# someone-in-somewhere/multimodal_rag

Hardware: AMD Instinct MI355X
Metric: chunks embedded/sec + queries/sec top_k=5 over 1M×768 at 1/2/4/8 GPUs (higher is better)
Workload: dtype f16

## Files before the change

multimodal_rag_amd/csrc/search_qsw.hip:

```cpp
#include "search_shared.h"

#include <type_traits>
#include <utility>

using namespace mmrag;

namespace mmrag_impl {

namespace {

template <typename F, int... I>
__device__ __forceinline__ void static_for_impl(F &&f, std::integer_sequence<int, I...>) {
    (f(std::integral_constant<int, I>{}), ...);
}
template <int N, typename F>
__device__ __forceinline__ void static_for(F &&f) {
    static_for_impl(f, std::make_integer_sequence<int, N>{});
}

constexpr int QSW_XCH = 2048 + 64;
constexpr int qsw_lists_bytes(int K, int MS) { return K * (MS == 32 ? 2 : 4) * QS_QROWS * 8; }

constexpr SlabRing qsw_ring(int NK, int K, int MS) {
#if defined(MMRAG_QSW_RING16)
    if (MS == 16 && NK % (MMRAG_QSW_RING16 / 10) == 0) return SlabRing{MMRAG_QSW_RING16 / 10, MMRAG_QSW_RING16 % 10};
#endif
    return slab_ring(NK, qsw_lists_bytes(K, MS) + QSW_XCH);
}

#define MMRAG_QSW_S32(MNEMONIC, QC, C00, C01, C10, C11, ACC)                                                  \
    asm volatile("v_xad_u32 %[t], %[lo], %[xc], %[st]\n\t"                                                    \
                 "ds_read_b128 %[n0], %[t] offset:%[o0]\n\t"                                                  \
                 "ds_read_b128 %[n1], %[t] offset:%[o1]\n\t" MNEMONIC " %[c00], %[a0], %[q0], " C00 "\n\t"    \
                 MNEMONIC " %[c01], %[a0], %[q1], " C01 "\n\t" MNEMONIC " %[c10], %[a1], %[q0], " C10 "\n\t"  \
                 MNEMONIC " %[c11], %[a1], %[q1], " C11 "\n\t"                                                \
                 "s_waitcnt lgkmcnt(0)"                                                                       \
                 : [c00] ACC(c00), [c01] ACC(c01), [c10] ACC(c10), [c11] ACC(c11), [n0] "=&v"(n0),            \
                   [n1] "=&v"(n1), [t] "=&v"(tmp)                                                             \
                 : [a0] "v"(a0), [a1] "v"(a1), [q0] QC(q0), [q1] QC(q1), [lo] "v"(lo), [st] "s"(st),          \
                   [xc] "i"(XC), [o0] "i"(OFF0), [o1] "i"(OFF1))

template <int DT, bool QA, bool FIRST, int XC, int OFF0, int OFF1, typename FT>
__device__ __forceinline__ void qsw_stmt32(f32x16_t &c00, f32x16_t &c01, f32x16_t &c10, f32x16_t &c11, const FT a0,
                                           const FT a1, const FT q0, const FT q1, FT &n0, FT &n1, const unsigned lo,
                                           const unsigned st) {
    unsigned tmp;
    if constexpr (FIRST) {
        static_assert(QA, "the first k-step's Q fragments live in the accumulator file");
        if constexpr (DT == MMRAG_F16) MMRAG_QSW_S32("v_mfma_f32_32x32x16_f16", "a", "0", "0", "0", "0", "=&v");
        else MMRAG_QSW_S32("v_mfma_f32_32x32x16_bf16", "a", "0", "0", "0", "0", "=&v");
    } else if constexpr (DT == MMRAG_F16) {
        if constexpr (QA) MMRAG_QSW_S32("v_mfma_f32_32x32x16_f16", "a", "%[c00]", "%[c01]", "%[c10]", "%[c11]", "+v");
        else MMRAG_QSW_S32("v_mfma_f32_32x32x16_f16", "v", "%[c00]", "%[c01]", "%[c10]", "%[c11]", "+v");
    } else {
        if constexpr (QA) MMRAG_QSW_S32("v_mfma_f32_32x32x16_bf16", "a", "%[c00]", "%[c01]", "%[c10]", "%[c11]", "+v");
        else MMRAG_QSW_S32("v_mfma_f32_32x32x16_bf16", "v", "%[c00]", "%[c01]", "%[c10]", "%[c11]", "+v");
    }
}

#define MMRAG_QSW_S16(MNEMONIC, QC, D0, D1, D2, D3, D4, D5, D6, D7, ACC)                                      \
    asm volatile(MNEMONIC " %[d0], %[a0], %[q0], " D0 "\n\t"                                                  \
                 "ds_read_b128 %[n0], %[ad] offset:%[o0]\n\t" MNEMONIC " %[d1], %[a0], %[q1], " D1 "\n\t"     \
                 "ds_read_b128 %[n1], %[ad] offset:%[o1]\n\t" MNEMONIC " %[d2], %[a0], %[q2], " D2 "\n\t"     \
                 MNEMONIC " %[d3], %[a0], %[q3], " D3 "\n\t" MNEMONIC " %[d4], %[a1], %[q0], " D4 "\n\t"      \
                 MNEMONIC " %[d5], %[a1], %[q1], " D5 "\n\t" MNEMONIC " %[d6], %[a1], %[q2], " D6 "\n\t"      \
                 MNEMONIC " %[d7], %[a1], %[q3], " D7 "\n\t"                                                  \
                 "s_waitcnt lgkmcnt(0)"                                                                       \
                 : [d0] ACC(d0), [d1] ACC(d1), [d2] ACC(d2), [d3] ACC(d3), [d4] ACC(d4), [d5] ACC(d5),        \
                   [d6] ACC(d6), [d7] ACC(d7), [n0] "=&v"(n0), [n1] "=&v"(n1)                                 \
                 : [a0] "v"(a0), [a1] "v"(a1), [q0] QC(q0), [q1] QC(q1), [q2] QC(q2), [q3] QC(q3),            \
                   [ad] "v"(adr), [o0] "i"(OFF0), [o1] "i"(OFF1))
#define MMRAG_QSW_S16_ACC(MNEMONIC, QC)                                                                       \
    MMRAG_QSW_S16(MNEMONIC, QC, "%[d0]", "%[d1]", "%[d2]", "%[d3]", "%[d4]", "%[d5]", "%[d6]", "%[d7]", "+v")
#define MMRAG_QSW_S16_FIRST(MNEMONIC, QC) MMRAG_QSW_S16(MNEMONIC, QC, "0", "0", "0", "0", "0", "0", "0", "0", "=&v")

template <int DT, bool QA, bool FIRST, int OFF0, int OFF1, typename FT>
__device__ __forceinline__ void qsw_stmt16(f32x4_t &d0, f32x4_t &d1, f32x4_t &d2, f32x4_t &d3, f32x4_t &d4,
                                           f32x4_t &d5, f32x4_t &d6, f32x4_t &d7, const FT a0, const FT a1,
                                           const FT q0, const FT q1, const FT q2, const FT q3, FT &n0, FT &n1,
                                           const unsigned adr) {
    if constexpr (FIRST) {
        static_assert(QA, "the first k-step's Q fragments live in the accumulator file");
        if constexpr (DT == MMRAG_F16) MMRAG_QSW_S16_FIRST("v_mfma_f32_16x16x32_f16", "a");
        else MMRAG_QSW_S16_FIRST("v_mfma_f32_16x16x32_bf16", "a");
    } else if constexpr (DT == MMRAG_F16) {
        if constexpr (QA) MMRAG_QSW_S16_ACC("v_mfma_f32_16x16x32_f16", "a");
        else MMRAG_QSW_S16_ACC("v_mfma_f32_16x16x32_f16", "v");
    } else {
        if constexpr (QA) MMRAG_QSW_S16_ACC("v_mfma_f32_16x16x32_bf16", "a");
        else MMRAG_QSW_S16_ACC("v_mfma_f32_16x16x32_bf16", "v");
    }
}

__device__ __forceinline__ void qsw_stage_addr(unsigned &a_lo, unsigned &a_hi, const unsigned lo, const unsigned st) {
    asm volatile("v_add_u32 %0, %2, %3\n\tv_xad_u32 %1, %2, 64, %3" : "=&v"(a_lo), "=&v"(a_hi) : "v"(lo), "s"(st));
}

__device__ __forceinline__ float max16_raw(float x0, float x1, float x2, float x3, float x4, float x5, float x6, float x7,
                                           float x8, float x9, float x10, float x11, float x12, float x13, float x14,
                                           float x15) {
    float r;
    asm("v_max3_f32 %0, %1, %2, %3\n\t"
        "v_max3_f32 %0, %0, %4, %5\n\t"
        "v_max3_f32 %0, %0, %6, %7\n\t"
        "v_max3_f32 %0, %0, %8, %9\n\t"
        "v_max3_f32 %0, %0, %10, %11\n\t"
        "v_max3_f32 %0, %0, %12, %13\n\t"
        "v_max3_f32 %0, %0, %14, %15\n\t"
        "v_max_f32 %0, %0, %16"
        : "=&v"(r)
        : "v"(x0), "v"(x1), "v"(x2), "v"(x3), "v"(x4), "v"(x5), "v"(x6), "v"(x7), "v"(x8), "v"(x9), "v"(x10), "v"(x11),
          "v"(x12), "v"(x13), "v"(x14), "v"(x15));
    return r;
}

constexpr int CP_SC1 = 16;

}

template <int DT, int NK, int K, int MS, bool NT>
__global__ __launch_bounds__(256, 1) void cosine_topk_walk_kernel(const KParams p) {
#if defined(__HIP_DEVICE_COMPILE__)
    using FT = typename FragType<DT>::T;
    static_assert(MS == 32 || MS == 16, "MFMA shape");
    constexpr int R = QS_TILE_ROWS;
    static_assert(R == 64, "statements are written for 64-row tiles");
    constexpr int RB = R / 32;
    constexpr int SLABB = R * SLAB;
    constexpr int NQB = MS == 32 ? 2 : 4;
    constexpr int QW = MS;
    constexpr int NSUB = 64 / QW;
    constexpr int NGRP = 16 / NSUB;
    constexpr SlabRing RING = qsw_ring(NK, K, MS);
    constexpr int G = RING.G, NST = RING.NST;
    constexpr int SPT = NK / G;
    constexpr int STAGE = G * SLABB;
    constexpr int PPS = G * RB;
    constexpr int KSTG = G * 4;
    constexpr int KST = MS == 32 ? NK * 4 : NK * 2;
    constexpr int QA_STEPS = 64 / NQB;
    constexpr int LISTS = qsw_lists_bytes(K, MS);
    constexpr int LOOK = (NST + 1 + SPT - 1) / SPT + 1;
    static_assert(NST >= 3 && NST * STAGE + LISTS + QSW_XCH <= 160 * 1024, "LDS");
    static_assert((NST - 1) * PPS <= 56, "vmcnt range");
    static_assert((G - 1) * SLABB + 48 * SLAB + 2048 < 65536, "ds_read immediate offset");
    static_assert(2 * PPS == KSTG, "one piece after every other statement");
    constexpr int LANDT = ((NST - 2) * PPS + 1 + SPT * PPS - 1) / (SPT * PPS);
    static_assert(LANDT >= 1 && LANDT * SPT * PPS - 1 >= (NST - 2) * PPS, "exchange pieces land before they are used");
    static_assert(LOOK <= 6, "ticket slots");

    __shared__ __attribute__((aligned(1024))) char smem[NST * STAGE + LISTS + QSW_XCH];
    float *lists = (float *)(smem + NST * STAGE);
    float *const gather_lds = (float *)(smem + NST * STAGE + LISTS);
    float *const poll_lds = (float *)(smem + NST * STAGE + LISTS + 1024);
    int *const tk_lds = (int *)(smem + NST * STAGE + LISTS + 2048);

    const int tid = threadIdx.x;
    const int lane = tid & 63;
    const int wave = __builtin_amdgcn_readfirstlane(tid >> 6);
    const int ql = lane & (QW - 1);
    const int sub = lane / QW;
    auto dev_dbg = [&](unsigned flag) -> bool {
#if defined(MMRAG_QSW_DEV)
        return (p.dbg & flag) != 0;
#else
        (void)flag;
        return false;
#endif
    };
    const unsigned long long t_entry = (p.dbg & DBG_QS_CLOCK) ? __builtin_amdgcn_s_memrealtime() : 0ull;

    const unsigned RBy = p.row_bytes;
    const int walkers = p.walkers;
    const int bx = (int)blockIdx.x % walkers;
    const int by = (int)blockIdx.x / walkers;
    const int q0 = by * QS_QROWS;
    const int p_static = p.p_static;
    auto pos_tile = [&](int pos) -> int {
        if (pos < p_static) return bx + pos * walkers;
        return p_static * walkers + (int)((unsigned)__builtin_amdgcn_readfirstlane(tk_lds[pos & 7]) - TICKET0);
    };

    unsigned c_off0;
    {
        const int row = (wave * RB) * 8 + (lane >> 3);
        c_off0 = (unsigned)row * RBy + (unsigned)(((lane & 7) ^ ((row >> 1) & 7)) * 16);
    }
    auto c_off = [&](int i) -> unsigned { return i == 0 ? c_off0 : (c_off0 ^ 64u) + 8u * RBy; };
    int is_pos = 0;
    int fill_tile = bx;
    __amdgpu_buffer_rsrc_t fill_rsrc;
    typedef __attribute__((address_space(3))) char *lds_char_t;
    const lds_char_t wave_lds = (lds_char_t)(lds_ptr_t)(smem + wave * (RB * 1024));
    lds_char_t stage_lds = wave_lds;
    auto fill_open = [&]() {
        const bool real = (unsigned)fill_tile < (unsigned)p.n_tiles && !dev_dbg(DBG_QS_NO_DMA);
        const long long row0 = real ? (dev_dbg(DBG_QS_DMA_L2) ? (long long)bx * R : (long long)fill_tile * R) : 0;
        const long long rows_left = p.n - row0;
        const unsigned c_bytes = real ? (unsigned)((rows_left < R ? rows_left : (long long)R) * (long long)RBy) : 0u;
        fill_rsrc = __builtin_amdgcn_make_buffer_rsrc((void *)(p.corpus + (size_t)row0 * RBy), 0, c_bytes, 0x00020000);
    };
    auto next_fill = [&](auto is_sg_c, int buf) {
        constexpr int IS_SG = decltype(is_sg_c)::value;
        if constexpr (IS_SG == 0) {
            if (is_pos != 0) fill_tile = pos_tile(is_pos);
            fill_open();
            ++is_pos;
        }
        stage_lds = wave_lds + buf * STAGE;
        asm volatile("" : "+s"(stage_lds));
    };
    unsigned koff = 0;
    auto issue_piece = [&](auto is_sg_c, auto pi_c) {
        constexpr int IS_SG = decltype(is_sg_c)::value, PI = decltype(pi_c)::value;
        constexpr int g = PI / RB, i = PI % RB;
        if constexpr (i == 0) asm volatile("s_movk_i32 %0, %1" : "=s"(koff) : "n"((IS_SG * G + g) * SLAB));
        __builtin_amdgcn_raw_ptr_buffer_load_lds(fill_rsrc, (lds_ptr_t)(stage_lds + g * SLABB + i * 1024), 16, c_off(i),
                                                 koff, 0, NT ? 2 : 0);
    };

    const bool any_tile = bx < p.n_tiles;
    if (any_tile)
        static_for<NST>([&](auto st_c) {
            constexpr int st = decltype(st_c)::value;
            next_fill(std::integral_constant<int, st % SPT>{}, st);
            static_for<PPS>([&](auto pi_c) { issue_piece(std::integral_constant<int, st % SPT>{}, pi_c); });
        });
    asm volatile("s_movk_i32 %0, %1" : "=s"(koff) : "n"(((NST - 1) % SPT) * G * SLAB));

    FT qf[NQB][KST];
    float thr[NQB];
    static_for<NQB>([&](auto qb_c) {
        constexpr int qb = decltype(qb_c)::value;
        const int qrow = q0 + wave * 64 + qb * QW + ql;
        const bool live = qrow < p.B;
        const char *src = p.q + (size_t)(live ? qrow : 0) * RBy + sub * 16;
#pragma unroll
        for (int s = 0; s < KST; ++s) {
            FT v = *(const FT *)(src + s * (16 * NSUB));
            if (!live) v = FT{};
            qf[qb][s] = v;
        }
        thr[qb] = !live ? INFINITY : NEG_INF;
    });
    float *const my_lists = lists + tid;
    auto lst_v = [&](int qb, int i) -> float & { return my_lists[(qb * 2 * K + i) * QS_QROWS]; };
    auto lst_r = [&](int qb, int i) -> int & { return *(int *)&my_lists[(qb * 2 * K + K + i) * QS_QROWS]; };
#pragma unroll
    for (int qb = 0; qb < NQB; ++qb)
#pragma unroll
        for (int i = 0; i < K; ++i) {
            lst_v(qb, i) = NEG_INF;
            lst_r(qb, i) = INT_MAX;
        }

    const int sw = (ql >> 1) & 7;
    const unsigned lane_off0 = (unsigned)(ql * SLAB + ((sub ^ sw) * 16));
    const unsigned lane_off64 = lane_off0 ^ 64u;
    const unsigned smem_base = (unsigned)(size_t)(lds_ptr_t)smem;

    auto lane_now = []() -> int {
        int l;
        asm volatile("v_mbcnt_lo_u32_b32 %0, -1, 0\n\tv_mbcnt_hi_u32_b32 %0, -1, %0" : "=v"(l));
        return l;
    };
    f32x16_t c32[MS == 32 ? 4 : 1];
    f32x4_t c16[MS == 16 ? 16 : 1];
    auto score = [&](auto qb_c, auto gi_c, int i) -> float {
        constexpr int qb = decltype(qb_c)::value, gi = decltype(gi_c)::value;
        if constexpr (MS == 32) return c32[(gi >> 2) * 2 + qb][4 * (gi & 3) + i];
        else return c16[gi * 4 + qb][i];
    };
    auto grp_row = [](int gi) -> int { return MS == 32 ? (gi >> 2) * 32 + 8 * (gi & 3) : gi * 16; };
    auto strike = [&](unsigned m0, unsigned m1, const int sub) {
        static_for<NQB>([&](auto qb_c) {
            static_for<NGRP>([&](auto gi_c) {
                constexpr int qb = decltype(qb_c)::value, gi = decltype(gi_c)::value;
                constexpr int r0 = MS == 32 ? (gi >> 2) * 32 + 8 * (gi & 3) : gi * 16;
                const unsigned m = (r0 < 32 ? m0 : m1) >> ((r0 & 31) + 4 * sub);
#pragma unroll
                for (int i = 0; i < 4; ++i) {
                    const bool ok = (m >> i) & 1u;
                    if constexpr (MS == 32) {
                        constexpr int a = (gi >> 2) * 2 + qb, e = 4 * (gi & 3);
                        c32[a][e + i] = ok ? c32[a][e + i] : NEG_INF;
                    } else {
                        c16[gi * 4 + qb][i] = ok ? c16[gi * 4 + qb][i] : NEG_INF;
                    }
                }
            });
        });
    };

    auto select = [&](auto qb_c, const int row_base, float *const my_lists) {
        auto lst_v = [&](int qb, int i) -> float & { return my_lists[(qb * 2 * K + i) * QS_QROWS]; };
        auto lst_r = [&](int qb, int i) -> int & { return *(int *)&my_lists[(qb * 2 * K + K + i) * QS_QROWS]; };
        constexpr int qb = decltype(qb_c)::value;
        auto max16 = [&](auto g0_c) -> float {
            constexpr int g0 = decltype(g0_c)::value;
            using G0 = std::integral_constant<int, g0>;
            using G1 = std::integral_constant<int, g0 + 1>;
            using G2 = std::integral_constant<int, g0 + 2>;
            using G3 = std::integral_constant<int, g0 + 3>;
            return max16_raw(score(qb_c, G0{}, 0), score(qb_c, G0{}, 1), score(qb_c, G0{}, 2), score(qb_c, G0{}, 3),
                             score(qb_c, G1{}, 0), score(qb_c, G1{}, 1), score(qb_c, G1{}, 2), score(qb_c, G1{}, 3),
                             score(qb_c, G2{}, 0), score(qb_c, G2{}, 1), score(qb_c, G2{}, 2), score(qb_c, G2{}, 3),
                             score(qb_c, G3{}, 0), score(qb_c, G3{}, 1), score(qb_c, G3{}, 2), score(qb_c, G3{}, 3));
        };
        float mx = max16(std::integral_constant<int, 0>{});
        if constexpr (NGRP == 8) mx = fmaxf(mx, max16(std::integral_constant<int, 4>{}));
        float t = thr[qb];
        if (__builtin_amdgcn_ballot_w64(mx >= t) == 0ull) return;
        constexpr int NE = NGRP * 4;
        float bar = t;
        if (__builtin_amdgcn_ballot_w64(t == NEG_INF) != 0ull) {
            float prev = INFINITY;
#pragma unroll
            for (int r = 0; r < K; ++r) {
                float m = NEG_INF;
                static_for<NGRP>([&](auto gi_c) {
                    const float x0 = score(qb_c, gi_c, 0), x1 = score(qb_c, gi_c, 1);
                    const float x2 = score(qb_c, gi_c, 2), x3 = score(qb_c, gi_c, 3);
                    const float y0 = x0 < prev ? x0 : NEG_INF, y1 = x1 < prev ? x1 : NEG_INF;
                    const float y2 = x2 < prev ? x2 : NEG_INF, y3 = x3 < prev ? x3 : NEG_INF;
                    m = fmaxf(m, fmaxf(fmaxf(y0, y1), fmaxf(y2, y3)));
                });
                prev = m;
            }
            bar = fmaxf(t, prev);
        }
        unsigned mask = 0;
        static_for<NE>([&](auto e_c) {
            constexpr int e = decltype(e_c)::value;
            mask |= score(qb_c, std::integral_constant<int, e / 4>{}, e % 4) >= bar ? (1u << e) : 0u;
        });
        TopList<K> L;
#pragma unroll
        for (int i = 0; i < K; ++i) {
            L.v[i] = lst_v(qb, i);
            L.r[i] = lst_r(qb, i);
        }
        constexpr int DENSE_AT = NE == 16 ? 8 : 12;
        if (__builtin_amdgcn_ballot_w64(__builtin_popcount(mask) > DENSE_AT) == 0ull) {
            while (__builtin_amdgcn_ballot_w64(mask != 0u) != 0ull) {
                const bool valid = mask != 0u;
                const unsigned e = (unsigned)__builtin_ctz(mask | (1u << (NE - 1)));
                mask &= mask - 1u;
                float lvl[NE];
                static_for<NE>([&](auto e_c) {
                    constexpr int x = decltype(e_c)::value;
                    lvl[x] = score(qb_c, std::integral_constant<int, x / 4>{}, x % 4);
                });
#pragma unroll
                for (int w = NE / 2, b = 0; w >= 1; w >>= 1, ++b) {
                    const bool bit = (e >> b) & 1u;
#pragma unroll
                    for (int i = 0; i < w; ++i) lvl[i] = bit ? lvl[2 * i + 1] : lvl[2 * i];
                }
                const float sc = lvl[0];
                const int row = MS == 32 ? (int)(((e >> 4) << 5) + (((e >> 2) & 3u) << 3) + (e & 3u))
                                         : (int)(((e >> 2) << 4) + (e & 3u));
                L.insert_strict_flat(valid && sc >= t ? sc : NEG_INF, row_base + row);
                t = fmaxf(t, L.v[K - 1]);
            }
        } else {
            static_for<NGRP>([&](auto gi_c) {
                constexpr int gi = decltype(gi_c)::value;
                const float a0 = score(qb_c, gi_c, 0), a1 = score(qb_c, gi_c, 1);
                const float a2 = score(qb_c, gi_c, 2), a3 = score(qb_c, gi_c, 3);
                if (__builtin_amdgcn_ballot_w64(fmaxf(fmaxf(a0, a1), fmaxf(a2, a3)) >= t) != 0ull) {
#pragma clang loop unroll(disable)
                    for (int i = 0; i < 4; ++i) {
                        const float s = i == 0 ? a0 : (i == 1 ? a1 : (i == 2 ? a2 : a3));
                        const bool pass = s >= t;
                        if (__builtin_amdgcn_ballot_w64(pass) != 0ull) {
                            L.insert_strict(pass ? s : NEG_INF, row_base + grp_row(gi) + i);
                            t = fmaxf(t, L.v[K - 1]);
                        }
                    }
                }
            });
        }
        float u = fmaxf(L.v[K - 1], __shfl_xor(L.v[K - 1], QW));
#pragma unroll
        for (int i = 0; i + 1 < K; ++i) u = fmaxf(u, fminf(L.v[i], __shfl_xor(L.v[K - 2 - i], QW)));
        if constexpr (NSUB == 4) u = fmaxf(u, __shfl_xor(u, 32));
        thr[qb] = fmaxf(t, u);
#pragma unroll
        for (int i = 0; i < K; ++i) {
            lst_v(qb, i) = L.v[i];
            lst_r(qb, i) = L.r[i];
        }
    };

    const bool seeding = p.pub_best != nullptr;
    const int n_resp = (QS_QROWS + walkers - 1) / walkers;
    auto publish_bests = [&](const int ql, const int sub, float *const my_lists) {
        auto lst_v = [&](int qb, int i) -> float & { return my_lists[(qb * 2 * K + i) * QS_QROWS]; };
        float *dst = p.pub_best + ((size_t)by * walkers + bx) * QS_QROWS + wave * 64 + ql;
        static_for<NQB>([&](auto qb_c) {
            constexpr int qb = decltype(qb_c)::value;
            float v = lst_v(qb, 0);
            v = fmaxf(v, __shfl_xor(v, QW));
            if constexpr (NSUB == 4) v = fmaxf(v, __shfl_xor(v, 32));
            if (sub == 0) __hip_atomic_store(dst + qb * QW, v, __ATOMIC_RELAXED, __HIP_MEMORY_SCOPE_AGENT);
        });
    };
    auto gather_issue = [&](int q) {
        const int ln = lane_now();
        const __amdgpu_buffer_rsrc_t rs = __builtin_amdgcn_make_buffer_rsrc(
            (void *)(p.pub_best + (size_t)by * walkers * QS_QROWS), 0, (unsigned)(walkers * QS_QROWS * 4), 0x00020000);
#pragma unroll
        for (int c = 0; c < 4; ++c)
            __builtin_amdgcn_raw_ptr_buffer_load_lds(rs, (lds_ptr_t)((char *)gather_lds + c * 256), 4,
                                                     (unsigned)(((c * 64 + ln) * QS_QROWS + q) * 4), 0, 0, CP_SC1);
    };
    auto compute_thr = [&](int q) {
        const int ln = lane_now();
        float v[4];
#pragma unroll
        for (int c = 0; c < 4; ++c) v[c] = (c * 64 + ln) < walkers ? gather_lds[c * 64 + ln] : NEG_INF;
        const float t = wave_kth_largest<K>(v[0], v[1], v[2], v[3], ln);
        if (ln == 0)
            __hip_atomic_store(p.pub_thr + (size_t)by * QS_QROWS + q, t, __ATOMIC_RELAXED, __HIP_MEMORY_SCOPE_AGENT);
    };
    auto poll_issue = [&]() {
        const __amdgpu_buffer_rsrc_t rs = __builtin_amdgcn_make_buffer_rsrc(
            (void *)(p.pub_thr + (size_t)by * QS_QROWS), 0, QS_QROWS * 4, 0x00020000);
        __builtin_amdgcn_raw_ptr_buffer_load_lds(rs, (lds_ptr_t)poll_lds, 16, (unsigned)(lane_now() * 16), 0, 0, CP_SC1);
    };
    auto poll_consume = [&](const int ql) {
        static_for<NQB>([&](auto qb_c) {
            constexpr int qb = decltype(qb_c)::value;
            thr[qb] = fmaxf(thr[qb], poll_lds[wave * 64 + qb * QW + ql]);
        });
    };
    constexpr int STEP = LANDT;
    const int span = n_resp * STEP + LANDT + 1;
    const int pub1 = span + 1 > 5 ? span + 1 : 5;
    auto polled_at = [&](int t) -> bool { return t >= 1 + LANDT && (t < pub1 + span + 4 || (t & 3) == 3); };
    const int quiet = pub1 + span + 4 + LANDT;

    unsigned long long t0c = 0, t0r = 0;
    if (p.dbg & DBG_QS_CLOCK) {
        t0c = __builtin_amdgcn_s_memtime();
        t0r = __builtin_amdgcn_s_memrealtime();
    }
    if (any_tile) {
        FT fa0, fa1, fb0, fb1;
        wait_vmcnt<(NST - 1) * PPS>();
        __builtin_amdgcn_s_barrier();
        {
            const char *st = smem + lane_off0;
            fa0 = *(const FT *)(st);
            fa1 = *(const FT *)(st + (MS == 32 ? 32 * SLAB : 16 * SLAB));
        }
        int cur_tile = bx;
        for (int ti = 0; (unsigned)cur_tile < (unsigned)p.n_tiles; ++ti) {
            unsigned adr_lo = 0, adr_hi = 0;
            if constexpr (MS == 16)
                qsw_stage_addr(adr_lo, adr_hi, lane_off0, smem_base + (unsigned)(((ti * SPT) % NST) * STAGE));
            unsigned tkv;
            const bool want_ticket = ti + LOOK >= p_static && wave == 0;
            if (want_ticket) {
                unsigned long long saved_exec;
                asm volatile("s_mov_b64 %1, exec\n\t"
                             "s_mov_b64 exec, 1\n\t"
                             "global_atomic_add %0, %2, %3, %4 sc0\n\t"
                             "s_mov_b64 exec, %1"
                             : "=&v"(tkv), "=&s"(saved_exec)
                             : "v"(0u), "v"(1u), "s"(p.tickets + by)
                             : "memory");
            }
            static_for<SPT>([&](auto sg_c) {
                constexpr int sg = decltype(sg_c)::value;
                const int it = ti * SPT + sg;
                const unsigned st_cur = smem_base + (unsigned)((it % NST) * STAGE);
                const unsigned st_nxt = smem_base + (unsigned)(((it + 1) % NST) * STAGE);
                static_for<KSTG>([&](auto j_c) {
                    constexpr int j = decltype(j_c)::value;
                    constexpr int g = j / 4, m = j % 4;
                    constexpr bool last = j == KSTG - 1;
                    constexpr int nj = last ? 0 : j + 1;
                    constexpr int ng = nj / 4, nm = nj % 4;
                    constexpr int slab = sg * G + g;
                    const unsigned st = last ? st_nxt : st_cur;
                    FT &x0 = (j & 1) ? fb0 : fa0, &x1 = (j & 1) ? fb1 : fa1;
                    FT &y0 = (j & 1) ? fa0 : fb0, &y1 = (j & 1) ? fa1 : fb1;
                    if constexpr (MS == 32) {
                        constexpr int ks = slab * 4 + m;
                        qsw_stmt32<DT, (ks < QA_STEPS), ks == 0, (nm & 1) * 32, ng * SLABB, ng * SLABB + 32 * SLAB, FT>(
                            c32[0], c32[1], c32[2], c32[3], x0, x1, qf[0][ks], qf[1][ks], y0, y1,
                            (nm & 2) ? lane_off64 : lane_off0, st);
                    } else {
                        constexpr int ks = slab * 2 + (m >> 1), rp = m & 1;
                        constexpr int o0 = ng * SLABB + (nm & 1) * (32 * SLAB);
                        if constexpr (last) qsw_stage_addr(adr_lo, adr_hi, lane_off0, st_nxt);
                        qsw_stmt16<DT, (ks < QA_STEPS), ks == 0, o0, o0 + 16 * SLAB, FT>(
                            c16[rp * 8 + 0], c16[rp * 8 + 1], c16[rp * 8 + 2], c16[rp * 8 + 3], c16[rp * 8 + 4],
                            c16[rp * 8 + 5], c16[rp * 8 + 6], c16[rp * 8 + 7], x0, x1, qf[0][ks], qf[1][ks], qf[2][ks],
                            qf[3][ks], y0, y1, (nm >> 1) ? adr_hi : adr_lo);
                    }
                    if constexpr (j == KSTG - 2) {
                        wait_vmcnt<(NST - 2) * PPS>();
                        if (!dev_dbg(DBG_QS_NO_BARRIER)) __builtin_amdgcn_s_barrier();
                        next_fill(std::integral_constant<int, (NST + sg) % SPT>{}, it % NST);
                    }
                    if constexpr (j == KSTG - 1)
                        issue_piece(std::integral_constant<int, (NST + sg) % SPT>{}, std::integral_constant<int, 0>{});
                    else if constexpr ((j & 1) == 1)
                        issue_piece(std::integral_constant<int, (NST + sg + SPT - 1) % SPT>{},
                                    std::integral_constant<int, (j + 1) / 2>{});
                });
            });
            asm volatile("s_nop 15\n\ts_nop 7");
            const long long row0 = (long long)cur_tile * R;
            if (row0 + R > p.n || p.alive_bits != nullptr) {
                const long long left = p.n - row0;
                unsigned m0 = left >= 32 ? 0xffffffffu : ((1u << (int)left) - 1u);
                unsigned m1 = left >= 64 ? 0xffffffffu : (left > 32 ? ((1u << (int)(left - 32)) - 1u) : 0u);
                if (p.alive_bits != nullptr) {
                    typedef const __attribute__((address_space(4))) uint32_t *scalar_words_t;
                    const scalar_words_t words = (scalar_words_t)p.alive_bits;
                    m0 &= words[row0 >> 5];
                    if (left > 32) m1 &= words[(row0 >> 5) + 1];
                }
                strike(m0, m1, lane_now() / QW);
            }
            const int ln = lane_now();
            const int ql_t = ln & (QW - 1), sub_t = ln / QW;
            float *const lists_t = lists + wave * 64 + ln;
            const int row_base = (int)row0 + 4 * sub_t;
            if (!(p.dbg & DBG_QS_NO_SELECT)) {
                static_for<NQB>([&](auto qb_c) { select(qb_c, row_base, lists_t); });
            } else {
                if constexpr (MS == 32) asm volatile("" ::"v"(c32[0]), "v"(c32[1]), "v"(c32[2]), "v"(c32[3]));
                else {
#pragma unroll
                    for (int e = 0; e < 16; ++e) asm volatile("" ::"v"(c16[e]));
                }
            }
            if (seeding && ti >= quiet) {
                if (((ti - LANDT) & 3) == 3) poll_consume(ql_t);
                if ((ti & 3) == 3 && wave == 0) poll_issue();
            } else if (seeding) {
                if (ti >= LANDT && polled_at(ti - LANDT)) poll_consume(ql_t);
                if (ti == 0 || ti == pub1) publish_bests(ql_t, sub_t, lists_t);
                if (wave == 0) {
                    const int rel = ti > pub1 ? ti - (pub1 + 1) : ti - 1;
                    const int jc = rel - LANDT, jg = rel;
                    if (jc >= 0 && jc % STEP == 0 && jc / STEP < n_resp && bx + (jc / STEP) * walkers < QS_QROWS)
                        compute_thr(bx + (jc / STEP) * walkers);
                    if (jg >= 0 && jg % STEP == 0 && jg / STEP < n_resp && bx + (jg / STEP) * walkers < QS_QROWS)
                        gather_issue(bx + (jg / STEP) * walkers);
                    if (polled_at(ti)) poll_issue();
                }
            }
            if ((p.dbg & DBG_QS_CLOCK) && p.stamps != nullptr && ti < 28 && wave == 0 && ln == 0)
                p.stamps[32 * blockIdx.x + 4 + ti] = __builtin_amdgcn_s_memrealtime();
            if (want_ticket) {
                wait_vmcnt<SPT * PPS>();
                unsigned long long saved_exec;
                const unsigned slot = (unsigned)(size_t)(lds_ptr_t)(tk_lds + ((ti + LOOK) & 7));
                asm volatile("s_mov_b64 %0, exec\n\t"
                             "s_mov_b64 exec, 1\n\t"
                             "ds_write_b32 %1, %2\n\t"
                             "s_mov_b64 exec, %0"
                             : "=&s"(saved_exec)
                             : "v"(slot), "v"(tkv)
                             : "memory");
            }
            cur_tile = pos_tile(ti + 1);
        }
    }
    const int tid_e = wave * 64 + lane_now();
    if ((p.dbg & DBG_QS_CLOCK) && p.stamps != nullptr && tid_e == 0) {
        p.stamps[32 * blockIdx.x] = __builtin_amdgcn_s_memtime() - t0c;
        p.stamps[32 * blockIdx.x + 1] = __builtin_amdgcn_s_memrealtime() - t0r;
        p.stamps[32 * blockIdx.x + 2] = t0r - t_entry;
        p.stamps[32 * blockIdx.x + 3] = t_entry;
    }
    __syncthreads();
    if (q0 + tid_e < p.B) {
        const int w = tid_e >> 6, qb = (tid_e / QW) & (NQB - 1), c = tid_e & (QW - 1);
        const float *la = lists + w * 64 + c + (qb * 2 * K) * QS_QROWS;
        TopList<K> m;
#pragma unroll
        for (int i = 0; i < K; ++i) {
            m.v[i] = la[i * QS_QROWS];
            m.r[i] = __float_as_int(la[(K + i) * QS_QROWS]);
        }
        for (int s = 1; s < NSUB; ++s) {
            const float *lb = la + s * QW;
            for (int i = 0; i < K; ++i) {
                const float x = lb[i * QS_QROWS];
                const int xr = __float_as_int(lb[(K + i) * QS_QROWS]);
                if (xr == INT_MAX || !better(x, xr, m.v[K - 1], m.r[K - 1])) break;
                m.insert_ordered(x, xr);
            }
        }
        const size_t base = ((size_t)(q0 + tid_e) * p.n_lists + bx) * K;
#pragma unroll
        for (int i = 0; i < K; ++i) {
            p.cand_s[base + i] = m.v[i];
            p.cand_r[base + i] = m.r[i];
        }
        if (bx == 0 && p.n_lists > walkers) {
            const size_t seed = ((size_t)(q0 + tid_e) * p.n_lists + (p.n_lists - 1)) * K;
#pragma unroll
            for (int i = 0; i < K; ++i) {
                p.cand_s[seed + i] = NEG_INF;
                p.cand_r[seed + i] = INT_MAX;
            }
        }
    }
#endif
}

bool qsw_supported(int dtype, unsigned row_bytes, int K, int mfma) {
    if (dtype != MMRAG_F16 && dtype != MMRAG_BF16) return false;
    if (K != 5) return false;
    const unsigned nk = row_bytes / SLAB;
#if defined(MMRAG_QSW_DEV)
    return (mfma == 16 || mfma == 32) && row_bytes % SLAB == 0 && nk == 12 && dtype == MMRAG_F16;
#else
    return mfma == 16 && row_bytes % SLAB == 0 && (nk == 6 || nk == 8 || nk == 12);
#endif
}

template <int DT, int K, int MS>
static int qsw_launch_nk(const KParams &p, int grid, hipStream_t s) {
    const bool nt = !p.share_l2;
    switch (p.row_bytes / SLAB) {
#if !defined(MMRAG_QSW_DEV)
        case 6:
            if (nt) cosine_topk_walk_kernel<DT, 6, K, MS, true><<<grid, 256, 0, s>>>(p);
            else cosine_topk_walk_kernel<DT, 6, K, MS, false><<<grid, 256, 0, s>>>(p);
            break;
        case 8:
            if (nt) cosine_topk_walk_kernel<DT, 8, K, MS, true><<<grid, 256, 0, s>>>(p);
            else cosine_topk_walk_kernel<DT, 8, K, MS, false><<<grid, 256, 0, s>>>(p);
            break;
#endif
        case 12:
            if (nt) cosine_topk_walk_kernel<DT, 12, K, MS, true><<<grid, 256, 0, s>>>(p);
            else cosine_topk_walk_kernel<DT, 12, K, MS, false><<<grid, 256, 0, s>>>(p);
            break;
        default: return MMRAG_EUNSUPPORTED;
    }
    return MMRAG_OK;
}

int qsw_launch(int dtype, int K, int mfma, const KParams &p, int grid_x, int grid_y, hipStream_t s) {
    if (!qsw_supported(dtype, p.row_bytes, K, mfma)) return MMRAG_EUNSUPPORTED;
    KParams kp = p;
    kp.walkers = grid_x;
    kp.share_l2 = grid_y > 1;
    const int grid = grid_x * grid_y;
#if defined(MMRAG_QSW_DEV)
    if (mfma == 32) return qsw_launch_nk<MMRAG_F16, 5, 32>(kp, grid, s);
    return qsw_launch_nk<MMRAG_F16, 5, 16>(kp, grid, s);
#else
    if (dtype == MMRAG_F16) return qsw_launch_nk<MMRAG_F16, 5, 16>(kp, grid, s);
    return qsw_launch_nk<MMRAG_BF16, 5, 16>(kp, grid, s);
#endif
}

}
```

Before: 657,800.

## Park last-step Q fragments in LDS, rework tile selection and seeding schedule

For the 16x16 MFMA path, the last k-step Q fragments are stored to an LDS park area and read back during the last statements of each tile. This frees registers across the loop, at the cost of extra LDS traffic and ring sizing. Selection is rewritten to sort the tile's scores with a bitonic network when the first tile is processed or when many scores pass the threshold. Otherwise it keeps the incremental insert loop, replacing the old dense path. The seeding schedule now publishes the tile max instead of full lists on tile 0 and moves threshold consumption before selection, so tighter thresholds reach the select step one tile earlier.

```diff
diff --git a/multimodal_rag_amd/csrc/search_qsw.hip b/multimodal_rag_amd/csrc/search_qsw.hip
--- a/multimodal_rag_amd/csrc/search_qsw.hip
+++ b/multimodal_rag_amd/csrc/search_qsw.hip
@@ -20,13 +20,17 @@
 
 constexpr int QSW_XCH = 2048 + 64;
 constexpr int qsw_lists_bytes(int K, int MS) { return K * (MS == 32 ? 2 : 4) * QS_QROWS * 8; }
+constexpr int qsw_park_bytes(int MS) { return MS == 16 ? 4 * QS_QROWS * 16 : 0; }
 
 constexpr SlabRing qsw_ring(int NK, int K, int MS) {
 #if defined(MMRAG_QSW_RING16)
     if (MS == 16 && NK % (MMRAG_QSW_RING16 / 10) == 0) return SlabRing{MMRAG_QSW_RING16 / 10, MMRAG_QSW_RING16 % 10};
 #endif
-    return slab_ring(NK, qsw_lists_bytes(K, MS) + QSW_XCH);
-}
+    return slab_ring(NK, qsw_lists_bytes(K, MS) + QSW_XCH + qsw_park_bytes(MS));
+}
+static_assert(qsw_ring(12, 5, 16).G == 3 && qsw_ring(12, 5, 16).NST == 4, "ring at 1536-byte rows");
+static_assert(qsw_ring(8, 5, 16).G == 2 && qsw_ring(8, 5, 16).NST == 6, "ring at 1024-byte rows");
+static_assert(qsw_ring(6, 5, 16).G == 3 && qsw_ring(6, 5, 16).NST == 4, "ring at 768-byte rows");
 
 #define MMRAG_QSW_S32(MNEMONIC, QC, C00, C01, C10, C11, ACC)                                                  \
     asm volatile("v_xad_u32 %[t], %[lo], %[xc], %[st]\n\t"                                                    \
@@ -73,6 +77,54 @@
 #define MMRAG_QSW_S16_ACC(MNEMONIC, QC)                                                                       \
     MMRAG_QSW_S16(MNEMONIC, QC, "%[d0]", "%[d1]", "%[d2]", "%[d3]", "%[d4]", "%[d5]", "%[d6]", "%[d7]", "+v")
 #define MMRAG_QSW_S16_FIRST(MNEMONIC, QC) MMRAG_QSW_S16(MNEMONIC, QC, "0", "0", "0", "0", "0", "0", "0", "0", "=&v")
+
+#define MMRAG_QSW_S16_PARK(MNEMONIC, QC, X3, X4, X5, X6, X7, PA, ...)                                         \
+    asm volatile(MNEMONIC " %[d0], %[a0], %[q0], %[d0]\n\t"                                                   \
+                 "ds_read_b128 %[n0], %[ad] offset:%[o0]\n\t" MNEMONIC " %[d1], %[a0], %[q1], %[d1]\n\t"      \
+                 "ds_read_b128 %[n1], %[ad] offset:%[o1]\n\t" MNEMONIC " %[d2], %[a0], %[q2], %[d2]\n\t"      \
+                 X3 MNEMONIC " %[d3], %[a0], %[q3], %[d3]\n\t" X4 MNEMONIC " %[d4], %[a1], %[q0], %[d4]\n\t"  \
+                 X5 MNEMONIC " %[d5], %[a1], %[q1], %[d5]\n\t" X6 MNEMONIC " %[d6], %[a1], %[q2], %[d6]\n\t"  \
+                 X7 MNEMONIC " %[d7], %[a1], %[q3], %[d7]\n\t"                                                 \
+                 "s_waitcnt lgkmcnt(2)"                                                                       \
+                 : [d0] "+v"(d0), [d1] "+v"(d1), [d2] "+v"(d2), [d3] "+v"(d3), [d4] "+v"(d4), [d5] "+v"(d5),  \
+                   [d6] "+v"(d6), [d7] "+v"(d7), [n0] "=&v"(n0), [n1] "=&v"(n1), [px] "=&v"(px),              \
+                   [py] "=&v"(py), [pa] PA(pa)                                                                \
+                 : [a0] "v"(a0), [a1] "v"(a1), [q0] QC(q0), [q1] QC(q1), [q2] QC(q2), [q3] QC(q3),            \
+                   [ad] "v"(adr), [o0] "i"(OFF0), [o1] "i"(OFF1), [ox] "i"(POFF), [oy] "i"(POFF + PSTRIDE),   \
+                   ##__VA_ARGS__)
+#define MMRAG_QSW_S16_PARK_A(MNEMONIC, QC)                                                                    \
+    MMRAG_QSW_S16_PARK(MNEMONIC, QC, "v_mbcnt_lo_u32_b32 %[pa], -1, 0\n\t", "v_mbcnt_hi_u32_b32 %[pa], -1, %[pa]\n\t", \
+                       "v_lshl_add_u32 %[pa], %[pa], 4, %[pb]\n\t", "ds_read_b128 %[px], %[pa] offset:%[ox]\n\t", \
+                       "ds_read_b128 %[py], %[pa] offset:%[oy]\n\t", "=&v", [pb] "s"(pb))
+#define MMRAG_QSW_S16_PARK_B(MNEMONIC, QC)                                                                    \
+    MMRAG_QSW_S16_PARK(MNEMONIC, QC, "ds_read_b128 %[px], %[pa] offset:%[ox]\n\t",                             \
+                       "ds_read_b128 %[py], %[pa] offset:%[oy]\n\t", "", "", "", "+v")
+
+template <int DT, bool QA, bool SECOND, int OFF0, int OFF1, int PSTRIDE, typename FT>
+__device__ __forceinline__ void qsw_stmt16_park(f32x4_t &d0, f32x4_t &d1, f32x4_t &d2, f32x4_t &d3, f32x4_t &d4,
+                                                f32x4_t &d5, f32x4_t &d6, f32x4_t &d7, const FT a0, const FT a1,
+                                                const FT q0, const FT q1, const FT q2, const FT q3, FT &n0, FT &n1,
+                                                const unsigned adr, FT &px, FT &py, unsigned &pa, const unsigned pb) {
+    constexpr int POFF = SECOND ? 2 * PSTRIDE : 0;
+    if constexpr (!SECOND) {
+        if constexpr (DT == MMRAG_F16) {
+            if constexpr (QA) MMRAG_QSW_S16_PARK_A("v_mfma_f32_16x16x32_f16", "a");
+            else MMRAG_QSW_S16_PARK_A("v_mfma_f32_16x16x32_f16", "v");
+        } else {
+            if constexpr (QA) MMRAG_QSW_S16_PARK_A("v_mfma_f32_16x16x32_bf16", "a");
+            else MMRAG_QSW_S16_PARK_A("v_mfma_f32_16x16x32_bf16", "v");
+        }
+    } else {
+        (void)pb;
+        if constexpr (DT == MMRAG_F16) {
+            if constexpr (QA) MMRAG_QSW_S16_PARK_B("v_mfma_f32_16x16x32_f16", "a");
+            else MMRAG_QSW_S16_PARK_B("v_mfma_f32_16x16x32_f16", "v");
+        } else {
+            if constexpr (QA) MMRAG_QSW_S16_PARK_B("v_mfma_f32_16x16x32_bf16", "a");
+            else MMRAG_QSW_S16_PARK_B("v_mfma_f32_16x16x32_bf16", "v");
+        }
+    }
+}
 
 template <int DT, bool QA, bool FIRST, int OFF0, int OFF1, typename FT>
 __device__ __forceinline__ void qsw_stmt16(f32x4_t &d0, f32x4_t &d1, f32x4_t &d2, f32x4_t &d3, f32x4_t &d4,
@@ -140,8 +192,14 @@
     constexpr int KST = MS == 32 ? NK * 4 : NK * 2;
     constexpr int QA_STEPS = 64 / NQB;
     constexpr int LISTS = qsw_lists_bytes(K, MS);
+    constexpr int PARK = qsw_park_bytes(MS);
+    constexpr int PARK_OFF = NST * STAGE + LISTS + QSW_XCH;
+    constexpr int PARK_STRIDE = QS_QROWS * 16;
+    constexpr int NSTMT = NK * 4;
     constexpr int LOOK = (NST + 1 + SPT - 1) / SPT + 1;
-    static_assert(NST >= 3 && NST * STAGE + LISTS + QSW_XCH <= 160 * 1024, "LDS");
+    static_assert(NST >= 3 && NST * STAGE + LISTS + QSW_XCH + PARK <= 160 * 1024, "LDS");
+    static_assert(PARK_OFF % 16 == 0 && PARK_OFF + 3 * PARK_STRIDE < 65536 * 4, "parked fragments: aligned b128 reads");
+    static_assert(PARK == 0 || (KSTG >= 8 && NSTMT >= 8), "parked read-back placement");
     static_assert((NST - 1) * PPS <= 56, "vmcnt range");
     static_assert((G - 1) * SLABB + 48 * SLAB + 2048 < 65536, "ds_read immediate offset");
     static_assert(2 * PPS == KSTG, "one piece after every other statement");
@@ -149,7 +207,7 @@
     static_assert(LANDT >= 1 && LANDT * SPT * PPS - 1 >= (NST - 2) * PPS, "exchange pieces land before they are used");
     static_assert(LOOK <= 6, "ticket slots");
 
-    __shared__ __attribute__((aligned(1024))) char smem[NST * STAGE + LISTS + QSW_XCH];
+    __shared__ __attribute__((aligned(1024))) char smem[NST * STAGE + LISTS + QSW_XCH + PARK];
     float *lists = (float *)(smem + NST * STAGE);
     float *const gather_lds = (float *)(smem + NST * STAGE + LISTS);
     float *const poll_lds = (float *)(smem + NST * STAGE + LISTS + 1024);
@@ -243,6 +301,13 @@
         }
         thr[qb] = !live ? INFINITY : NEG_INF;
     });
+    if constexpr (PARK != 0) {
+        static_for<NQB>([&](auto qb_c) {
+            constexpr int qb = decltype(qb_c)::value;
+            *(FT *)(smem + PARK_OFF + qb * PARK_STRIDE + tid * 16) = qf[qb][KST - 1];
+        });
+        asm volatile("" ::: "memory");
+    }
     float *const my_lists = lists + tid;
     auto lst_v = [&](int qb, int i) -> float & { return my_lists[(qb * 2 * K + i) * QS_QROWS]; };
     auto lst_r = [&](int qb, int i) -> int & { return *(int *)&my_lists[(qb * 2 * K + K + i) * QS_QROWS]; };
@@ -271,7 +336,6 @@
         if constexpr (MS == 32) return c32[(gi >> 2) * 2 + qb][4 * (gi & 3) + i];
         else return c16[gi * 4 + qb][i];
     };
-    auto grp_row = [](int gi) -> int { return MS == 32 ? (gi >> 2) * 32 + 8 * (gi & 3) : gi * 16; };
     auto strike = [&](unsigned m0, unsigned m1, const int sub) {
         static_for<NQB>([&](auto qb_c) {
             static_for<NGRP>([&](auto gi_c) {
@@ -292,10 +356,7 @@
         });
     };
 
-    auto select = [&](auto qb_c, const int row_base, float *const my_lists) {
-        auto lst_v = [&](int qb, int i) -> float & { return my_lists[(qb * 2 * K + i) * QS_QROWS]; };
-        auto lst_r = [&](int qb, int i) -> int & { return *(int *)&my_lists[(qb * 2 * K + K + i) * QS_QROWS]; };
-        constexpr int qb = decltype(qb_c)::value;
+    auto blk_max = [&](auto qb_c) -> float {
         auto max16 = [&](auto g0_c) -> float {
             constexpr int g0 = decltype(g0_c)::value;
             using G0 = std::integral_constant<int, g0>;
@@ -309,39 +370,92 @@
         };
         float mx = max16(std::integral_constant<int, 0>{});
         if constexpr (NGRP == 8) mx = fmaxf(mx, max16(std::integral_constant<int, 4>{}));
+        return mx;
+    };
+
+    auto select = [&](auto qb_c, const int row_base, float *const my_lists, const bool first_tile) {
+        auto lst_v = [&](int qb, int i) -> float & { return my_lists[(qb * 2 * K + i) * QS_QROWS]; };
+        auto lst_r = [&](int qb, int i) -> int & { return *(int *)&my_lists[(qb * 2 * K + K + i) * QS_QROWS]; };
+        constexpr int qb = decltype(qb_c)::value;
+        const float mx = blk_max(qb_c);
         float t = thr[qb];
         if (__builtin_amdgcn_ballot_w64(mx >= t) == 0ull) return;
         constexpr int NE = NGRP * 4;
-        float bar = t;
-        if (__builtin_amdgcn_ballot_w64(t == NEG_INF) != 0ull) {
-            float prev = INFINITY;
+        auto hits = [&](const float bar) -> unsigned {
+            unsigned m = 0;
+            static_for<NE>([&](auto e_c) {
+                constexpr int e = decltype(e_c)::value;
+                m |= score(qb_c, std::integral_constant<int, e / 4>{}, e % 4) >= bar ? (1u << e) : 0u;
+            });
+            return m;
+        };
+        auto sorted_scores = [&](float (&v)[NE]) {
+            static_for<NE>([&](auto e_c) {
+                constexpr int e = decltype(e_c)::value;
+                v[e] = score(qb_c, std::integral_constant<int, e / 4>{}, e % 4);
+            });
+#pragma unroll
+            for (int pw = 1; pw < NE; pw *= 2)
+#pragma unroll
+                for (int kk = pw; kk >= 1; kk /= 2)
+#pragma unroll
+                    for (int j = kk % pw; j <= NE - 1 - kk; j += 2 * kk)
+#pragma unroll
+                        for (int i = 0; i <= (kk - 1 < NE - j - kk - 1 ? kk - 1 : NE - j - kk - 1); ++i)
+                            if ((i + j) / (2 * pw) == (i + j + kk) / (2 * pw)) {
+                                const float hi = fmaxf(v[i + j], v[i + j + kk]), lo = fminf(v[i + j], v[i + j + kk]);
+                                v[i + j] = hi;
+                                v[i + j + kk] = lo;
+                            }
+        };
+        constexpr int MANY = 4;
+        const unsigned mask0 = hits(t);
+        TopList<K> L;
+        if (first_tile || __builtin_amdgcn_ballot_w64(__builtin_popcount(mask0) >= MANY) != 0ull) {
+            float v[NE];
+            sorted_scores(v);
+            float cv[K];
+            int cr[K];
+            unsigned used = 0;
 #pragma unroll
             for (int r = 0; r < K; ++r) {
-                float m = NEG_INF;
-                static_for<NGRP>([&](auto gi_c) {
-                    const float x0 = score(qb_c, gi_c, 0), x1 = score(qb_c, gi_c, 1);
-                    const float x2 = score(qb_c, gi_c, 2), x3 = score(qb_c, gi_c, 3);
-                    const float y0 = x0 < prev ? x0 : NEG_INF, y1 = x1 < prev ? x1 : NEG_INF;
-                    const float y2 = x2 < prev ? x2 : NEG_INF, y3 = x3 < prev ? x3 : NEG_INF;
-                    m = fmaxf(m, fmaxf(fmaxf(y0, y1), fmaxf(y2, y3)));
+                unsigned m = 0;
+                static_for<NE>([&](auto e_c) {
+                    constexpr int e = decltype(e_c)::value;
+                    m |= score(qb_c, std::integral_constant<int, e / 4>{}, e % 4) == v[r] ? (1u << e) : 0u;
                 });
-                prev = m;
-            }
-            bar = fmaxf(t, prev);
-        }
-        unsigned mask = 0;
-        static_for<NE>([&](auto e_c) {
-            constexpr int e = decltype(e_c)::value;
-            mask |= score(qb_c, std::integral_constant<int, e / 4>{}, e % 4) >= bar ? (1u << e) : 0u;
-        });
-        TopList<K> L;
-#pragma unroll
-        for (int i = 0; i < K; ++i) {
-            L.v[i] = lst_v(qb, i);
-            L.r[i] = lst_r(qb, i);
-        }
-        constexpr int DENSE_AT = NE == 16 ? 8 : 12;
-        if (__builtin_amdgcn_ballot_w64(__builtin_popcount(mask) > DENSE_AT) == 0ull) {
+                m &= ~used;
+                const unsigned e = (unsigned)__builtin_ctz(m | (1u << (NE - 1)));
+                used |= 1u << e;
+                const int row = MS == 32 ? (int)(((e >> 4) << 5) + (((e >> 2) & 3u) << 3) + (e & 3u))
+                                         : (int)(((e >> 2) << 4) + (e & 3u));
+                const bool ok = v[r] >= t && v[r] > NEG_INF;
+                cv[r] = ok ? v[r] : NEG_INF;
+                cr[r] = ok ? row_base + row : INT_MAX;
+            }
+            if (first_tile) {
+#pragma unroll
+                for (int r = 0; r < K; ++r) {
+                    L.v[r] = cv[r];
+                    L.r[r] = cr[r];
+                }
+            } else {
+#pragma unroll
+                for (int i = 0; i < K; ++i) {
+                    L.v[i] = lst_v(qb, i);
+                    L.r[i] = lst_r(qb, i);
+                }
+#pragma unroll
+                for (int r = 0; r < K; ++r) L.insert_strict_flat(cv[r], cr[r]);
+            }
+            t = fmaxf(t, L.v[K - 1]);
+        } else {
+            unsigned mask = mask0;
+#pragma unroll
+            for (int i = 0; i < K; ++i) {
+                L.v[i] = lst_v(qb, i);
+                L.r[i] = lst_r(qb, i);
+            }
             while (__builtin_amdgcn_ballot_w64(mask != 0u) != 0ull) {
                 const bool valid = mask != 0u;
                 const unsigned e = (unsigned)__builtin_ctz(mask | (1u << (NE - 1)));
@@ -363,23 +477,6 @@
                 L.insert_strict_flat(valid && sc >= t ? sc : NEG_INF, row_base + row);
                 t = fmaxf(t, L.v[K - 1]);
             }
-        } else {
-            static_for<NGRP>([&](auto gi_c) {
-                constexpr int gi = decltype(gi_c)::value;
-                const float a0 = score(qb_c, gi_c, 0), a1 = score(qb_c, gi_c, 1);
-                const float a2 = score(qb_c, gi_c, 2), a3 = score(qb_c, gi_c, 3);
-                if (__builtin_amdgcn_ballot_w64(fmaxf(fmaxf(a0, a1), fmaxf(a2, a3)) >= t) != 0ull) {
-#pragma clang loop unroll(disable)
-                    for (int i = 0; i < 4; ++i) {
-                        const float s = i == 0 ? a0 : (i == 1 ? a1 : (i == 2 ? a2 : a3));
-                        const bool pass = s >= t;
-                        if (__builtin_amdgcn_ballot_w64(pass) != 0ull) {
-                            L.insert_strict(pass ? s : NEG_INF, row_base + grp_row(gi) + i);
-                            t = fmaxf(t, L.v[K - 1]);
-                        }
-                    }
-                }
-            });
         }
         float u = fmaxf(L.v[K - 1], __shfl_xor(L.v[K - 1], QW));
 #pragma unroll
@@ -406,6 +503,16 @@
             if (sub == 0) __hip_atomic_store(dst + qb * QW, v, __ATOMIC_RELAXED, __HIP_MEMORY_SCOPE_AGENT);
         });
     };
+    auto publish_tile_max = [&](const int ql, const int sub) {
+        float *dst = p.pub_best + ((size_t)by * walkers + bx) * QS_QROWS + wave * 64 + ql;
+        static_for<NQB>([&](auto qb_c) {
+            constexpr int qb = decltype(qb_c)::value;
+            float v = thr[qb] == INFINITY ? NEG_INF : blk_max(qb_c);
+            v = fmaxf(v, __shfl_xor(v, QW));
+            if constexpr (NSUB == 4) v = fmaxf(v, __shfl_xor(v, 32));
+            if (sub == 0) __hip_atomic_store(dst + qb * QW, v, __ATOMIC_RELAXED, __HIP_MEMORY_SCOPE_AGENT);
+        });
+    };
     auto gather_issue = [&](int q) {
         const int ln = lane_now();
         const __amdgpu_buffer_rsrc_t rs = __builtin_amdgcn_make_buffer_rsrc(
@@ -438,7 +545,7 @@
     constexpr int STEP = LANDT;
     const int span = n_resp * STEP + LANDT + 1;
     const int pub1 = span + 1 > 5 ? span + 1 : 5;
-    auto polled_at = [&](int t) -> bool { return t >= 1 + LANDT && (t < pub1 + span + 4 || (t & 3) == 3); };
+    auto polled_at = [&](int t) -> bool { return t >= LANDT && (t < pub1 + span + 4 || (t & 3) == 3); };
     const int quiet = pub1 + span + 4 + LANDT;
 
     unsigned long long t0c = 0, t0r = 0;
@@ -448,6 +555,8 @@
     }
     if (any_tile) {
         FT fa0, fa1, fb0, fb1;
+        FT pq0, pq1, pq2, pq3;
+        unsigned park_adr;
         wait_vmcnt<(NST - 1) * PPS>();
         __builtin_amdgcn_s_barrier();
         {
@@ -496,10 +605,26 @@
                         constexpr int ks = slab * 2 + (m >> 1), rp = m & 1;
                         constexpr int o0 = ng * SLABB + (nm & 1) * (32 * SLAB);
                         if constexpr (last) qsw_stage_addr(adr_lo, adr_hi, lane_off0, st_nxt);
-                        qsw_stmt16<DT, (ks < QA_STEPS), ks == 0, o0, o0 + 16 * SLAB, FT>(
-                            c16[rp * 8 + 0], c16[rp * 8 + 1], c16[rp * 8 + 2], c16[rp * 8 + 3], c16[rp * 8 + 4],
-                            c16[rp * 8 + 5], c16[rp * 8 + 6], c16[rp * 8 + 7], x0, x1, qf[0][ks], qf[1][ks], qf[2][ks],
-                            qf[3][ks], y0, y1, (nm >> 1) ? adr_hi : adr_lo);
+                        constexpr int tix = slab * 4 + m;
+                        if constexpr (PARK != 0 && (tix == NSTMT - 6 || tix == NSTMT - 5)) {
+                            static_assert(j < KSTG - 2 && ks < KST - 1, "read-back statement");
+                            constexpr bool second = tix == NSTMT - 5;
+                            qsw_stmt16_park<DT, (ks < QA_STEPS), second, o0, o0 + 16 * SLAB, PARK_STRIDE, FT>(
+                                c16[rp * 8 + 0], c16[rp * 8 + 1], c16[rp * 8 + 2], c16[rp * 8 + 3], c16[rp * 8 + 4],
+                                c16[rp * 8 + 5], c16[rp * 8 + 6], c16[rp * 8 + 7], x0, x1, qf[0][ks], qf[1][ks],
+                                qf[2][ks], qf[3][ks], y0, y1, (nm >> 1) ? adr_hi : adr_lo, second ? pq2 : pq0,
+                                second ? pq3 : pq1, park_adr, smem_base + (unsigned)(PARK_OFF + wave * 1024));
+                        } else if constexpr (PARK != 0 && ks == KST - 1) {
+                            qsw_stmt16<DT, false, false, o0, o0 + 16 * SLAB, FT>(
+                                c16[rp * 8 + 0], c16[rp * 8 + 1], c16[rp * 8 + 2], c16[rp * 8 + 3], c16[rp * 8 + 4],
+                                c16[rp * 8 + 5], c16[rp * 8 + 6], c16[rp * 8 + 7], x0, x1, pq0, pq1, pq2, pq3, y0, y1,
+                                (nm >> 1) ? adr_hi : adr_lo);
+                        } else {
+                            qsw_stmt16<DT, (ks < QA_STEPS), ks == 0, o0, o0 + 16 * SLAB, FT>(
+                                c16[rp * 8 + 0], c16[rp * 8 + 1], c16[rp * 8 + 2], c16[rp * 8 + 3], c16[rp * 8 + 4],
+                                c16[rp * 8 + 5], c16[rp * 8 + 6], c16[rp * 8 + 7], x0, x1, qf[0][ks], qf[1][ks],
+                                qf[2][ks], qf[3][ks], y0, y1, (nm >> 1) ? adr_hi : adr_lo);
+                        }
                     }
                     if constexpr (j == KSTG - 2) {
                         wait_vmcnt<(NST - 2) * PPS>();
@@ -531,8 +656,19 @@
             const int ql_t = ln & (QW - 1), sub_t = ln / QW;
             float *const lists_t = lists + wave * 64 + ln;
             const int row_base = (int)row0 + 4 * sub_t;
+            if (seeding && ti >= quiet) {
+                if (((ti - LANDT) & 3) == 3) poll_consume(ql_t);
+            } else if (seeding) {
+                if (ti >= LANDT && polled_at(ti - LANDT)) poll_consume(ql_t);
+                if (ti == 0) publish_tile_max(ql_t, sub_t);
+                if (wave == 0) {
+                    const int jc = (ti > pub1 ? ti - (pub1 + 1) : ti) - LANDT;
+                    if (jc >= 0 && jc % STEP == 0 && jc / STEP < n_resp && bx + (jc / STEP) * walkers < QS_QROWS)
+                        compute_thr(bx + (jc / STEP) * walkers);
+                }
+            }
             if (!(p.dbg & DBG_QS_NO_SELECT)) {
-                static_for<NQB>([&](auto qb_c) { select(qb_c, row_base, lists_t); });
+                static_for<NQB>([&](auto qb_c) { select(qb_c, row_base, lists_t, ti == 0); });
             } else {
                 if constexpr (MS == 32) asm volatile("" ::"v"(c32[0]), "v"(c32[1]), "v"(c32[2]), "v"(c32[3]));
                 else {
@@ -541,17 +677,12 @@
                 }
             }
             if (seeding && ti >= quiet) {
-                if (((ti - LANDT) & 3) == 3) poll_consume(ql_t);
                 if ((ti & 3) == 3 && wave == 0) poll_issue();
             } else if (seeding) {
-                if (ti >= LANDT && polled_at(ti - LANDT)) poll_consume(ql_t);
-                if (ti == 0 || ti == pub1) publish_bests(ql_t, sub_t, lists_t);
+                if (ti == pub1) publish_bests(ql_t, sub_t, lists_t);
                 if (wave == 0) {
-                    const int rel = ti > pub1 ? ti - (pub1 + 1) : ti - 1;
-                    const int jc = rel - LANDT, jg = rel;
-                    if (jc >= 0 && jc % STEP == 0 && jc / STEP < n_resp && bx + (jc / STEP) * walkers < QS_QROWS)
-                        compute_thr(bx + (jc / STEP) * walkers);
-                    if (jg >= 0 && jg % STEP == 0 && jg / STEP < n_resp && bx + (jg / STEP) * walkers < QS_QROWS)
+                    const int jg = ti > pub1 ? ti - (pub1 + 1) : ti;
+                    if (jg % STEP == 0 && jg / STEP < n_resp && bx + (jg / STEP) * walkers < QS_QROWS)
                         gather_issue(bx + (jg / STEP) * walkers);
                     if (polled_at(ti)) poll_issue();
                 }
```

Result: faster. 674,700 (median of 6 runs) (+2.6%).
